# DeepBlender/DeepDenoiser

Hardware: AMD Instinct MI355X
Metric: train tiles/sec (128x128x32ch U-Net KPCN) (higher is better)
Workload: dtype bf16; 1 GPU; BASELINE config 2: U-Net [64,96,128]x4 + 5x5 KernelPrediction + 3-scale MultiScalePrediction, 32-channel render-pass stack, 128x128 tiles, full training step (fwd+SMAPE loss+bwd+Adam); global_batch=128, parallelism=dp1, hipgraph=True, inputs=resident in HBM

## Files before the change

deepdenoiser_amd/csrc/dd_compose_stream.h:

```cpp
#pragma once
#include "dd_common.h"
#include <type_traits>

namespace {

typedef __attribute__((ext_vector_type(16))) float f32x16_t;
typedef __attribute__((ext_vector_type(2))) unsigned int cs_u32x2;

template <typename T> __device__ __forceinline__ f32x16_t mma32(uint4 a, uint4 b, f32x16_t c);
template <> __device__ __forceinline__ f32x16_t mma32<bf16_t>(uint4 a, uint4 b, f32x16_t c) {
  return __builtin_amdgcn_mfma_f32_32x32x16_bf16(__builtin_bit_cast(bf16x8_t, a), __builtin_bit_cast(bf16x8_t, b), c, 0, 0, 0);
}
template <> __device__ __forceinline__ f32x16_t mma32<f16_t>(uint4 a, uint4 b, f32x16_t c) {
  return __builtin_amdgcn_mfma_f32_32x32x16_f16(__builtin_bit_cast(f16x8_t, a), __builtin_bit_cast(f16x8_t, b), c, 0, 0, 0);
}

typedef __attribute__((ext_vector_type(4))) unsigned int cs_u32x4;
template <typename T> __device__ __forceinline__ f32x16_t mma32_zero(uint4 a, uint4 b);
template <> __device__ __forceinline__ f32x16_t mma32_zero<bf16_t>(uint4 a, uint4 b) {
  f32x16_t d;
  const cs_u32x4 av = {a.x, a.y, a.z, a.w}, bv = {b.x, b.y, b.z, b.w};
  asm volatile("v_mfma_f32_32x32x16_bf16 %0, %1, %2, 0" : "=&v"(d) : "v"(av), "v"(bv));
  return d;
}
template <> __device__ __forceinline__ f32x16_t mma32_zero<f16_t>(uint4 a, uint4 b) {
  f32x16_t d;
  const cs_u32x4 av = {a.x, a.y, a.z, a.w}, bv = {b.x, b.y, b.z, b.w};
  asm volatile("v_mfma_f32_32x32x16_f16 %0, %1, %2, 0" : "=&v"(d) : "v"(av), "v"(bv));
  return d;
}

template <typename T> __device__ __forceinline__ void unpack2(uint32_t w, float& lo, float& hi);
template <> __device__ __forceinline__ void unpack2<bf16_t>(uint32_t w, float& lo, float& hi) { lo = __uint_as_float(w << 16); hi = __uint_as_float(w & 0xffff0000u); }
template <> __device__ __forceinline__ void unpack2<f16_t>(uint32_t w, float& lo, float& hi) { unpack_f16x2(w, lo, hi); }
template <typename T> __device__ __forceinline__ uint32_t packo(float lo, float hi) {
  uint32_t w = pack2<T>(lo, hi);
  asm("" : "+v"(w));
  return w;
}
template <typename T> struct One;
template <> struct One<bf16_t> { static constexpr uint32_t v = 0x3f80u; };
template <> struct One<f16_t> { static constexpr uint32_t v = 0x3c00u; };

__device__ __forceinline__ float dpp_xor1(float v) { return __int_as_float(__builtin_amdgcn_update_dpp(0, __float_as_int(v), 0xB1, 0xF, 0xF, true)); }
__device__ __forceinline__ void both_halves(float v, float& lower, float& upper) {
  const cs_u32x2 r = __builtin_amdgcn_permlane32_swap(__float_as_uint(v), __float_as_uint(v), false, false);
  lower = __uint_as_float(r[0]); upper = __uint_as_float(r[1]);
}

constexpr int PIXB = 48;

struct Unit { int b, yb0, yb1, xs, xe, fx0; };

template <typename P>
__device__ __forceinline__ void decode_unit(const P& p, int u, Unit& U) {
  const int j = u % p.nb, t = u / p.nb;
  const int st = t % p.n_strips;
  U.b = t / p.n_strips;
  U.yb0 = j * p.BH; U.yb1 = min(p.H, U.yb0 + p.BH);
  U.xs = st * p.SO; U.xe = min(p.W, U.xs + p.SO);
  U.fx0 = p.n_strips > 1 ? U.xs - 4 : 0;
}

struct Cursor {
  int urel, i;
  Unit U;
  template <typename P>
  __device__ __forceinline__ void init(const P& p, int u0, int nunits, int V) {
    urel = V >= 0 ? V / p.VB : -1 - ((-V - 1) / p.VB);
    i = V - urel * p.VB;
    U = Unit{0, 0, 0, 0, 0, 0};
    if (urel >= 0 && urel < nunits) decode_unit(p, u0 + urel, U);
  }
  template <typename P>
  __device__ __forceinline__ void advance(const P& p, int u0, int nunits, int rows) {
    i += rows;
    while (i >= p.VB) {
      i -= p.VB;
      ++urel;
      if (urel >= 0 && urel < nunits) decode_unit(p, u0 + urel, U);
    }
  }
};

__device__ __forceinline__ int sfl(int v) { return __builtin_amdgcn_readfirstlane(v); }
__device__ __forceinline__ int opaque(int v) { asm volatile("" : "+v"(v)); return v; }
__device__ __forceinline__ int posmod(int v, int d) { const int m = v % d; return m < 0 ? m + d : m; }

template <typename T> __device__ __forceinline__ float split3(float v, int e) {
  const float hi = Elem<T>::to_f32(Elem<T>::from_f32(v));
  const float mid = Elem<T>::to_f32(Elem<T>::from_f32(v - hi));
  const float lo = Elem<T>::to_f32(Elem<T>::from_f32(v - hi - mid));
  return e == 0 ? hi : e == 1 ? mid : lo;
}

}
```

deepdenoiser_amd/csrc/dd_compose_stream.hip:

```cpp
#include "dd_compose_stream.h"

#ifdef CS_PROFILE
__device__ unsigned long long cs_phase[4][8];
#define CSP_DECL() unsigned long long csp_last = __builtin_readcyclecounter(); const bool csp_on = blockIdx.x == 0 && t == 0 && lane == 0
#define CSP(i) do { const unsigned long long now_ = __builtin_readcyclecounter(); if (csp_on) cs_phase[LAYER][i] += now_ - csp_last; csp_last = now_; } while (0)
extern "C" int dd_debug_cs_phases(unsigned long long* out32, int reset) {
  if (out32) (void)hipMemcpyFromSymbol(out32, HIP_SYMBOL(cs_phase), sizeof(unsigned long long) * 32);
  if (reset) { unsigned long long z[32] = {0}; (void)hipMemcpyToSymbol(HIP_SYMBOL(cs_phase), z, sizeof(z)); }
  return 0;
}
#else
#define CSP_DECL()
#define CSP(i)
#endif


namespace {

constexpr int KS_MAX = 16;
constexpr int AUX_BYTES = 16 + 3 * 1024;

struct CsP {
  const float* small; const float* fine; float* out;
  const float* w_in; const float* b_in; const float* w_res[4]; const float* b_res[4]; const float* w_out; const float* b_out;
  void* save_act[5]; void* save_wl; void* save_netin;
  int ld_small, ld_fine, ld_out, ld_act[5], ld_wl, ld_netin;
  int N, H, W;
  int FW, R, TPR;
  int n_strips, SO;
  int BH, nb, VB;
  int units;
};

template <typename T>
__device__ __forceinline__ void stage_weights(char* img, char* aux, const CsP& p, int tid) {
  for (int i = tid; i < 4 * KS_MAX * 64 * 8; i += 1024) {
    const int e = i & 7, ln = (i >> 3) & 63, c = (i >> 9) & (KS_MAX - 1), l = i >> 13;
    const int m = ln & 31, g = 2 * c + (ln >> 5);
    float v = 0.f;
    if (m < 24) {
      if (g < 27) v = p.w_res[l][((g / 3) * 24 + 8 * (g % 3) + e) * 24 + m];
      else if (g == 27) { if (e < 3) v = split3<T>(p.b_res[l][m], e); }
    }
    reinterpret_cast<T*>(img)[i] = Elem<T>::from_f32(v);
  }
  T* ax = reinterpret_cast<T*>(aux);
  for (int i = tid; i < 8 + 3 * 512; i += 1024) {
    float v = 0.f;
    if (i < 8) v = i < 3 ? 1.f : 0.f;
    else {
      const int j = i - 8, e = j & 7, ln = (j >> 3) & 63, which = j >> 9;
      const int m = ln & 31, h = ln >> 5;
      if (which == 0) { if (m == 0) v = p.w_out[e < 4 ? 4 * h + e : 8 + 4 * h + e - 4]; }
      else if (which == 1) { if (m == 0) v = e < 4 ? p.w_out[16 + 4 * h + e] : (e < 7 && h == 0) ? split3<T>(p.b_out[0], e - 4) : 0.f; }
      else if (m < 24) v = e < 3 ? p.w_in[((h ? 0 : 3) + e) * 24 + m] : (e < 6 && h == 0) ? split3<T>(p.b_in[m], e - 3) : 0.f;
    }
    ax[i] = Elem<T>::from_f32(v);
  }
}

template <typename T, int LAYER, bool SAVE, int NPRE>
__device__ __forceinline__ void cs_role(const CsP& p, char* smem, char* aux, int ring_bytes, int t, int lane, int u0, int nunits, int steps) {
  constexpr bool RESIDUAL = LAYER == 1 || LAYER == 3;
  constexpr bool FINAL = LAYER == 3;
  constexpr int KS = 14;
  constexpr uint32_t ONE = One<T>::v, ONE2 = ONE | (ONE << 16);
  const int R = p.R, TPR = p.TPR, FW = p.FW, VB = p.VB;
  const int n = lane & 31, h = lane >> 5;
  const int r = t / TPR, xc = t - r * TPR;
  const bool has_task = t < R * TPR;
  const int x = xc * 32 + n;
  const int pitch = (FW + 2) * PIXB, rp = R * pitch;
  const int D0 = 3 * R + 2, D1 = 2 * R + 2, D4 = 3 * R + 2;
  const int off1 = D0 * pitch, off2 = off1 + D1 * pitch, off3 = off2 + D1 * pitch, off4 = off3 + D1 * pitch;
  const int Din = LAYER == 0 ? D0 : D1;
  const int Dres = LAYER == 1 ? D0 : D4;
  const int in_bytes = Din * pitch, out_bytes = D1 * pitch, res_bytes = Dres * pitch, raw_bytes = D4 * pitch;
  char* rin = smem + (LAYER == 0 ? 0 : LAYER == 1 ? off1 : LAYER == 2 ? off2 : off3);
  char* rout = smem + (LAYER == 0 ? off1 : LAYER == 1 ? off2 : off3);
  char* rres = smem + (LAYER == 1 ? 0 : off4);

  uint4 wa[KS];
#pragma unroll
  for (int c = 0; c < KS; ++c) wa[c] = *reinterpret_cast<const uint4*>(smem + ((LAYER * KS_MAX + c) * 64 + lane) * 16);
  __syncthreads();
  for (int i = threadIdx.x; i < ring_bytes / 16; i += 1024) reinterpret_cast<uint4*>(smem)[i] = uint4{0u, 0u, 0u, 0u};

  const int H = p.H, W = p.W, h2 = H >> 1, w2 = W >> 1;
  const int lag = (LAYER + 1) * (R + 1);
  const int total_rows = nunits * VB;
  const int s_beg = has_task ? (lag - r + R - 1) / R : steps, s_end = has_task ? (total_rows + lag - r + R - 1) / R : steps;
  Cursor cur;
  cur.init(p, u0, nunits, r - lag);
  int o_in = posmod(r - lag, Din) * pitch, o_out = posmod(r - lag, D1) * pitch, o_res = posmod(r - lag, Dres) * pitch, o_raw = posmod(r - lag, D4) * pitch;
  auto wrap_add = [](int o, int add, int bytes) { o += add; return o >= bytes ? o - bytes : o; };
  const int xo = x * PIXB + h * 16;
  const int a4c = h ? x * PIXB : x * PIXB + 128;
  const int a13c = h ? (int)(aux - rin) : x * PIXB + 128;
  const int wr = (x + 1) * PIXB + h * 8;
  int ybase = 0, pixb = 0;
  bool col_in = false, col_own = false, cols_all_in = false;
  auto unit_values = [&](const Cursor& c, int& yb, int& pb, bool& ci, bool& co, bool& call) {
    const int gx = c.U.fx0 + x;
    yb = c.U.yb0 - 4;
    ci = (unsigned)gx < (unsigned)W;
    co = ci && gx >= c.U.xs && gx < c.U.xe;
    pb = c.U.b * H * W + (ci ? gx : 0);
    call = c.U.fx0 + xc * 32 >= 0 && c.U.fx0 + xc * 32 + 32 <= W;
  };
  unit_values(cur, ybase, pixb, col_in, col_own, cols_all_in);

  Cursor c0;
  int o0 = 0, ybase0 = 0, pixb0 = 0, pix0 = 0;
  bool col_in0 = false, col_own0 = false, cols_all_in0 = false, in0 = false, own0 = false, row_in0 = false;
  float xin[3] = {0.f, 0.f, 0.f};
  const int s0_end = has_task ? (total_rows - r + R - 1) / R : 0;
  auto load_x0 = [&](int s_next) {
    in0 = false; own0 = false; row_in0 = false;
    if (s_next < s0_end) {
      const int y = ybase0 + c0.i;
      row_in0 = (unsigned)y < (unsigned)H;
      in0 = row_in0 && col_in0;
      own0 = in0 && col_own0 && y >= c0.U.yb0 && y < c0.U.yb1;
      const int cy = row_in0 ? y : 0;
      pix0 = pixb0 + cy * W;
      const int cx = pix0 - (c0.U.b * H + cy) * W;
      const float* src = h ? p.small + (size_t)((c0.U.b * h2 + (cy >> 1)) * w2 + (cx >> 1)) * p.ld_small : p.fine + (size_t)pix0 * p.ld_fine;
#ifdef CS_EXP_NO_STAGE0_LOADS
      xin[0] = (float)pix0; xin[1] = 1.f; xin[2] = 0.5f;
      (void)src;
#else
      xin[0] = src[0]; xin[1] = src[1]; xin[2] = src[2];
#endif
    }
  };
  if (LAYER == 0) {
    c0.init(p, u0, nunits, r);
    o0 = posmod(r, D0) * pitch;
    unit_values(c0, ybase0, pixb0, col_in0, col_own0, cols_all_in0);
    load_x0(0);
  }

  f32x16_t acc;
  auto conv_part_n = [&](auto pre_t) {
    constexpr bool pre = decltype(pre_t)::value;
    constexpr int C0 = pre ? 0 : NPRE, C1 = pre ? NPRE : KS;
    const int o_m1 = o_in == 0 ? in_bytes - pitch : o_in - pitch;
    const int o_p1 = o_in + pitch == in_bytes ? 0 : o_in + pitch;
    const char* q0 = rin + xo + o_m1;
    const char* q1 = rin + xo + 16 + o_in;
    const char* q2 = rin + xo + o_p1;
    const char* q4 = rin + a4c + (h ? o_in : o_m1);
    const char* q13 = rin + a13c + (h ? 0 : o_p1);
    f32x16_t c_init = {0.f, 0.f, 0.f, 0.f, 0.f, 0.f, 0.f, 0.f, 0.f, 0.f, 0.f, 0.f, 0.f, 0.f, 0.f, 0.f};
    if (RESIDUAL && pre) {
      const char* qr = rres + o_res + wr;
      uint2 rv[3];
#pragma unroll
      for (int b = 0; b < 3; ++b) rv[b] = *reinterpret_cast<const uint2*>(qr + b * 16);
#pragma unroll
      for (int b = 0; b < 3; ++b) {
        float r0, r1, r2, r3;
        unpack2<T>(rv[b].x, r0, r1); unpack2<T>(rv[b].y, r2, r3);
        c_init[4 * b] = r0; c_init[4 * b + 1] = r1; c_init[4 * b + 2] = r2; c_init[4 * b + 3] = r3;
      }
    }
    constexpr int BATCH = 6;
#pragma unroll
    for (int c0_ = C0; c0_ < C1; c0_ += BATCH) {
      uint4 bf[BATCH];
#pragma unroll
      for (int c = c0_; c < c0_ + BATCH && c < C1; ++c) {
        const char* a = c < 4 ? q0 + 32 * c : c == 4 ? q4 : c < 9 ? q1 + 32 * (c - 5) : c < 13 ? q2 + 32 * (c - 9) : q13;
#ifdef CS_EXP_NO_LDSREAD
        bf[c - c0_] = uint4{(uint32_t)x, (uint32_t)c, 0u, 0u};
#else
        bf[c - c0_] = *reinterpret_cast<const uint4*>(a);
#endif
      }
      __builtin_amdgcn_sched_barrier(0);
#pragma unroll
      for (int c = c0_; c < c0_ + BATCH && c < C1; ++c) {
#ifdef CS_EXP_NO_MFMA
        acc[c] = ((pre && c == 0) ? c_init[c] : acc[c]) + __uint_as_float(bf[c - c0_].x ^ wa[c].x);
#else
        acc = mma32<T>(wa[c], bf[c - c0_], (pre && c == 0) ? c_init : acc);
#endif
      }
      __builtin_amdgcn_sched_barrier(0);
    }
    if (pre && NPRE == 0) acc = c_init;
  };

  bool act = 0 >= s_beg && 0 < s_end;
  if (act) conv_part_n(std::true_type());

  CSP_DECL();
  for (int s = 0; s < steps; ++s) {
    CSP(0);
#ifndef CS_EXP_NO_BARRIER
    __syncthreads();
#endif
    CSP(1);
    if (LAYER == 0) {
      if (s < s0_end) {
        const uint4 w0 = *reinterpret_cast<const uint4*>(aux + 16 + 2048 + lane * 16);
        const uint4 bx = {pack2<T>(xin[0], xin[1]), pack2<T>(xin[2], h ? 0.f : 1.f), h ? 0u : ONE2, 0u};
        const f32x16_t z = {0.f, 0.f, 0.f, 0.f, 0.f, 0.f, 0.f, 0.f, 0.f, 0.f, 0.f, 0.f, 0.f, 0.f, 0.f, 0.f};
        const f32x16_t a0 = mma32<T>(w0, bx, z);
        char* o = rin + o0 + wr;
        const bool in_now = in0, own_now = own0, all_in = row_in0 && cols_all_in0;
        const int pix_now = pix0;
        if (SAVE && own_now && p.save_netin) {
          T* d = reinterpret_cast<T*>(p.save_netin) + (size_t)pix_now * p.ld_netin + (h ? 0 : 3);
#pragma unroll
          for (int e = 0; e < 3; ++e) d[e] = Elem<T>::from_f32(xin[e]);
          if (!h) { d[3] = Elem<T>::from_f32(0.f); d[4] = Elem<T>::from_f32(0.f); }
        }
        uint2 pk[3];
#pragma unroll
        for (int b = 0; b < 3; ++b) {
          pk[b].x = relu_bf16x2(packo<T>(a0[4 * b], a0[4 * b + 1]));
          pk[b].y = relu_bf16x2(packo<T>(a0[4 * b + 2], a0[4 * b + 3]));
        }
        if (!all_in) {
#pragma unroll
          for (int b = 0; b < 3; ++b) { pk[b].x = in_now ? pk[b].x : 0u; pk[b].y = in_now ? pk[b].y : 0u; }
        }
#pragma unroll
        for (int b = 0; b < 3; ++b) {
          *reinterpret_cast<uint2*>(o + b * 16) = pk[b];
          if (SAVE && own_now && p.save_act[0])
            *reinterpret_cast<uint2*>(reinterpret_cast<char*>(p.save_act[0]) + ((size_t)pix_now * p.ld_act[0] + 8 * b + 4 * h) * 2) = pk[b];
        }
      }
      c0.i += R;
      if (c0.i >= VB) {
        c0.i -= R;
        c0.advance(p, u0, nunits, R);
        unit_values(c0, ybase0, pixb0, col_in0, col_own0, cols_all_in0);
      }
      o0 = wrap_add(o0, rp, D0 * pitch);
      load_x0(s + 1);
    }
    CSP(2);
    if (act) {
      const int y = ybase + cur.i;
      const bool row_in = (unsigned)y < (unsigned)H;
      const bool all_in = row_in && cols_all_in;
      const bool inside = row_in && col_in;
      const bool own = inside && col_own && y >= cur.U.yb0 && y < cur.U.yb1;
      const int cy = row_in ? y : 0;
      const int pix = pixb + cy * W;
      float f3[3] = {0.f, 0.f, 0.f}, s3[3] = {0.f, 0.f, 0.f};
      if (FINAL) {
#ifndef CS_EXP_NO_TAIL_LOADS
        const int cx = pix - (cur.U.b * H + cy) * W;
        const float* fr = p.fine + (size_t)(pix + (h - (cy & 1)) * W) * p.ld_fine;
        const float* sp = p.small + (size_t)((cur.U.b * h2 + (cy >> 1)) * w2 + (cx >> 1)) * p.ld_small;
#pragma unroll
        for (int c = 0; c < 3; ++c) { f3[c] = fr[c]; s3[c] = sp[c]; }
#endif
      }
      conv_part_n(std::false_type());
      CSP(4);
      uint4 wo1 = {0u, 0u, 0u, 0u}, wo2 = {0u, 0u, 0u, 0u};
      if (FINAL) {
        wo1 = *reinterpret_cast<const uint4*>(aux + 16 + lane * 16);
        wo2 = *reinterpret_cast<const uint4*>(aux + 16 + 1024 + lane * 16);
      }
      uint2 pk[3];
#pragma unroll
      for (int b = 0; b < 3; ++b) {
        pk[b].x = packo<T>(acc[4 * b], acc[4 * b + 1]);
        pk[b].y = packo<T>(acc[4 * b + 2], acc[4 * b + 3]);
      }
      if (!FINAL) {
        if (LAYER == 1) {
          char* o4 = smem + off4 + o_raw + wr;
          if (!all_in) {
#pragma unroll
            for (int b = 0; b < 3; ++b) { pk[b].x = inside ? pk[b].x : 0u; pk[b].y = inside ? pk[b].y : 0u; }
          }
#pragma unroll
          for (int b = 0; b < 3; ++b) {
            *reinterpret_cast<uint2*>(o4 + b * 16) = pk[b];
            if (SAVE && own && p.save_act[2])
              *reinterpret_cast<uint2*>(reinterpret_cast<char*>(p.save_act[2]) + ((size_t)pix * p.ld_act[2] + 8 * b + 4 * h) * 2) = pk[b];
          }
        }
#pragma unroll
        for (int b = 0; b < 3; ++b) { pk[b].x = relu_bf16x2(pk[b].x); pk[b].y = relu_bf16x2(pk[b].y); }
        if (LAYER != 1 && !all_in) {
#pragma unroll
          for (int b = 0; b < 3; ++b) { pk[b].x = inside ? pk[b].x : 0u; pk[b].y = inside ? pk[b].y : 0u; }
        }
        char* o = rout + o_out + wr;
#pragma unroll
        for (int b = 0; b < 3; ++b) {
          *reinterpret_cast<uint2*>(o + b * 16) = pk[b];
          if (SAVE && LAYER != 1 && own && p.save_act[LAYER + 1])
            *reinterpret_cast<uint2*>(reinterpret_cast<char*>(p.save_act[LAYER + 1]) + ((size_t)pix * p.ld_act[LAYER + 1] + 8 * b + 4 * h) * 2) = pk[b];
        }
      } else {
#ifdef CS_EXP_NO_TAIL
        if (own && h == 0 && pk[0].x == 0x12345u) p.out[(size_t)pix * p.ld_out] = 1.f;
#else
        if (SAVE && own && p.save_act[4]) {
#pragma unroll
          for (int b = 0; b < 3; ++b)
            *reinterpret_cast<uint2*>(reinterpret_cast<char*>(p.save_act[4]) + ((size_t)pix * p.ld_act[4] + 8 * b + 4 * h) * 2) = pk[b];
        }
        const f32x16_t z = {0.f, 0.f, 0.f, 0.f, 0.f, 0.f, 0.f, 0.f, 0.f, 0.f, 0.f, 0.f, 0.f, 0.f, 0.f, 0.f};
        f32x16_t a2 = mma32<T>(wo1, uint4{pk[0].x, pk[0].y, pk[1].x, pk[1].y}, z);
        a2 = mma32<T>(wo2, uint4{pk[2].x, pk[2].y, ONE2, ONE}, a2);
        const uint32_t wlp = pack2<T>(fmaxf(a2[0], 0.f), 0.f);
        float wlv, unused;
        unpack2<T>(wlp, wlv, unused);
        const float wgt = 1.f / (1.f + __expf(-wlv));
        float res[3];
#pragma unroll
        for (int c = 0; c < 3; ++c) {
          const float pair = f3[c] + dpp_xor1(f3[c]);
          float p_lo, p_hi, f_lo, f_hi;
          both_halves(pair, p_lo, p_hi);
          both_halves(f3[c], f_lo, f_hi);
          const float low = 0.25f * (p_lo + p_hi);
          const float fme = (cy & 1) ? f_hi : f_lo;
          res[c] = fme - wgt * low + wgt * s3[c];
        }
        if (own && h == 0) {
          float* o = p.out + (size_t)pix * p.ld_out;
#pragma unroll
          for (int c = 0; c < 3; ++c) o[c] = res[c];
          if (SAVE && p.save_wl) reinterpret_cast<uint16_t*>(p.save_wl)[(size_t)pix * p.ld_wl] = (uint16_t)(wlp & 0xffffu);
        }
#endif
      }
    }
    CSP(5);
    cur.i += R;
    if (cur.i >= VB) {
      cur.i -= R;
      cur.advance(p, u0, nunits, R);
      unit_values(cur, ybase, pixb, col_in, col_own, cols_all_in);
    }
    o_in = wrap_add(o_in, rp, in_bytes);
    if (!FINAL) o_out = wrap_add(o_out, rp, out_bytes);
    if (RESIDUAL) o_res = wrap_add(o_res, rp, res_bytes);
    if (LAYER == 1) o_raw = wrap_add(o_raw, rp, raw_bytes);
    act = s + 1 >= s_beg && s + 1 < s_end;
    if (act) conv_part_n(std::true_type());
    CSP(6);
  }
}

template <typename T, bool SAVE, bool R1>
__global__ __launch_bounds__(1024) void compose_stream_fwd_kernel(const CsP p) {
  extern __shared__ __attribute__((aligned(16))) char smem[];
  const int tid = threadIdx.x, lane = tid & 63, wave = sfl(tid >> 6);
  const int rows = 12 * p.R + 10;
  const int ring_bytes = rows * (p.FW + 2) * PIXB;
  char* aux = smem + ring_bytes;
  stage_weights<T>(smem, aux, p, tid);
  const int G = gridDim.x, g = blockIdx.x;
  const int u0 = (int)(((long)p.units * g) / G), u1 = (int)(((long)p.units * (g + 1)) / G);
  const int nunits = u1 - u0;
  const int steps = nunits > 0 ? (nunits * p.VB + 4 * (p.R + 1) + p.R - 1) / p.R : 0;
  const int layer = wave >> 2, t = wave & 3;
  __syncthreads();
  const int r = t / p.TPR;
#define CS_ROLE(L)                                                                                   \
  do {                                                                                               \
    if (R1 || r == 0) cs_role<T, L, SAVE, 9>(p, smem, aux, ring_bytes, t, lane, u0, nunits, steps);  \
    else if (r == 1) cs_role<T, L, SAVE, 4>(p, smem, aux, ring_bytes, t, lane, u0, nunits, steps);   \
    else cs_role<T, L, SAVE, 0>(p, smem, aux, ring_bytes, t, lane, u0, nunits, steps);               \
  } while (0)
  if (layer == 0) CS_ROLE(0);
  else if (layer == 1) CS_ROLE(1);
  else if (layer == 2) CS_ROLE(2);
  else CS_ROLE(3);
#undef CS_ROLE
}

}

extern "C" int dd_compose_stream_plan(int N, int H, int W, int cus, int* out8) {
  if (N <= 0 || H <= 0 || W <= 0 || cus <= 0 || !out8) return DD_ERR_INVALID;
  int n_strips = 1, SO = W, FW = ((W + 31) / 32) * 32;
  if (W > 128) {
    for (n_strips = 2;; ++n_strips) {
      SO = (W + n_strips - 1) / n_strips;
      SO += SO & 1;
      FW = ((SO + 8 + 31) / 32) * 32;
      if (FW <= 128) break;
    }
  }
  const int R = FW == 32 ? 4 : FW == 64 ? 2 : 1;
  long best = -1; int bestBH = 0;
  for (int d = 1; d <= 16; ++d) {
    int BH = (H + d - 1) / d;
    BH = ((BH + 3) / 4) * 4;
    if (BH < 4) BH = 4;
    const int nb = (H + BH - 1) / BH;
    const long units = (long)N * n_strips * nb;
    const long G = units < cus ? units : cus;
    const long per = (units + G - 1) / G;
    const long cost = per * (BH + 8) + 4 * (R + 1);
    if (best < 0 || cost < best) { best = cost; bestBH = BH; }
  }
  const int nb = (H + bestBH - 1) / bestBH;
  out8[0] = FW; out8[1] = R; out8[2] = FW / 32; out8[3] = n_strips; out8[4] = SO; out8[5] = bestBH; out8[6] = nb; out8[7] = bestBH + 8;
  return DD_OK;
}

int dd_compose_stream_fwd_launch(const dd_compose_args* a, hipStream_t s) {
  CsP p;
  p.small = a->small; p.fine = a->fine; p.out = a->out;
  p.w_in = a->w_in; p.b_in = a->b_in; p.w_out = a->w_out; p.b_out = a->b_out;
  for (int l = 0; l < 4; ++l) { p.w_res[l] = a->w_res[l]; p.b_res[l] = a->b_res[l]; }
  bool save = a->save_wl != nullptr;
  for (int i = 0; i < 5; ++i) { p.save_act[i] = a->save_act[i]; p.ld_act[i] = a->ld_act[i]; save = save || a->save_act[i]; }
  p.save_wl = a->save_wl; p.ld_wl = a->ld_wl;
  p.save_netin = a->save_netin; p.ld_netin = a->ld_netin; save = save || a->save_netin;
  p.ld_small = a->ld_small; p.ld_fine = a->ld_fine; p.ld_out = a->ld_out;
  p.N = a->N; p.H = a->H; p.W = a->W;
  DD_REQUIRE((long)a->N * a->H * a->W < (1l << 31) / 64, "dd_compose_net_fwd: N * H * W = %ld pixels exceed the 32-bit offsets of the kernel", (long)a->N * a->H * a->W);
  const int cus = dd_device_cus();
  int g8[8];
  if (dd_compose_stream_plan(a->N, a->H, a->W, cus, g8) != DD_OK) return DD_ERR_INVALID;
  p.FW = g8[0]; p.R = g8[1]; p.TPR = g8[2]; p.n_strips = g8[3]; p.SO = g8[4]; p.BH = g8[5]; p.nb = g8[6]; p.VB = g8[7];
  p.units = a->N * p.n_strips * p.nb;
  const int grid = p.units < cus ? p.units : cus;
  const int lds = (12 * p.R + 10) * (p.FW + 2) * PIXB + AUX_BYTES;
#define CS_LAUNCH(T, SV, R1)                                                                          \
  do {                                                                                                \
    dd_allow_max_lds(reinterpret_cast<const void*>(compose_stream_fwd_kernel<T, SV, R1>));            \
    hipLaunchKernelGGL((compose_stream_fwd_kernel<T, SV, R1>), dim3(grid), dim3(1024), lds, s, p);    \
  } while (0)
#define CS_LAUNCH_R(T, SV) do { if (p.R == 1) CS_LAUNCH(T, SV, true); else CS_LAUNCH(T, SV, false); } while (0)
  if (a->dtype == DD_BF16) { if (save) CS_LAUNCH_R(bf16_t, true); else CS_LAUNCH_R(bf16_t, false); }
  else { if (save) CS_LAUNCH_R(f16_t, true); else CS_LAUNCH_R(f16_t, false); }
#undef CS_LAUNCH_R
#undef CS_LAUNCH
  DD_LAUNCH_CHECK();
  return DD_OK;
}
```

Baseline: 16110 tiles/s.

## Widen activation saves via permlane swap and prefetch tail loads earlier

Activation saves now go through a helper that uses permlane32_swap so each half-wave writes one 16-byte store instead of two 8-byte stores per pixel for the first two channel blocks. The final layer's fine and small image loads are issued before the pre-part of the next step's convolution, so their global-memory latency overlaps with MFMA work. The final layer's pre-part batch size drops to 3, and the act[4] save moves after the tail computation. Compile-time experiment macros to disable saves are also added. Register pressure rises because the f3/s3 values are now live across the loop.

```diff
diff --git a/deepdenoiser_amd/csrc/dd_compose_stream.h b/deepdenoiser_amd/csrc/dd_compose_stream.h
--- a/deepdenoiser_amd/csrc/dd_compose_stream.h
+++ b/deepdenoiser_amd/csrc/dd_compose_stream.h
@@ -50,6 +50,20 @@
 
 constexpr int PIXB = 48;
 
+__device__ __forceinline__ void store_pixel24(bool pred, char* px, int h, uint2 pk0, uint2 pk1, uint2 pk2) {
+  const cs_u32x2 sx = __builtin_amdgcn_permlane32_swap(pk0.x, pk1.x, false, false);
+  const cs_u32x2 sy = __builtin_amdgcn_permlane32_swap(pk0.y, pk1.y, false, false);
+  if (pred) {
+#ifdef CS_EXP_NARROW_SAVES
+    *reinterpret_cast<uint2*>(px + 8 * h) = pk0;
+    *reinterpret_cast<uint2*>(px + 16 + 8 * h) = pk1;
+#else
+    *reinterpret_cast<uint4*>(px + 16 * h) = uint4{sx[0], sy[0], sx[1], sy[1]};
+#endif
+    *reinterpret_cast<uint2*>(px + 32 + 8 * h) = pk2;
+  }
+}
+
 struct Unit { int b, yb0, yb1, xs, xe, fx0; };
 
 template <typename P>
diff --git a/deepdenoiser_amd/csrc/dd_compose_stream.hip b/deepdenoiser_amd/csrc/dd_compose_stream.hip
--- a/deepdenoiser_amd/csrc/dd_compose_stream.hip
+++ b/deepdenoiser_amd/csrc/dd_compose_stream.hip
@@ -12,6 +12,12 @@
 #else
 #define CSP_DECL()
 #define CSP(i)
+#endif
+
+#ifdef CS_EXP_NO_SAVES
+#define CS_SAVING(word) ((word) == 0x7fc12345u)
+#else
+#define CS_SAVING(word) true
 #endif
 
 
@@ -165,7 +171,7 @@
         c_init[4 * b] = r0; c_init[4 * b + 1] = r1; c_init[4 * b + 2] = r2; c_init[4 * b + 3] = r3;
       }
     }
-    constexpr int BATCH = 6;
+    constexpr int BATCH = (pre && FINAL) ? 3 : 6;
 #pragma unroll
     for (int c0_ = C0; c0_ < C1; c0_ += BATCH) {
       uint4 bf[BATCH];
@@ -192,8 +198,25 @@
     if (pre && NPRE == 0) acc = c_init;
   };
 
+  float f3[3] = {0.f, 0.f, 0.f}, s3[3] = {0.f, 0.f, 0.f};
+  auto request_tail = [&]() {
+#ifndef CS_EXP_NO_TAIL_LOADS
+    const int y = ybase + cur.i;
+    const int cy = (unsigned)y < (unsigned)H ? y : 0;
+    const int pix = pixb + cy * W;
+    const int cx = pix - (cur.U.b * H + cy) * W;
+    const float* fr = p.fine + (size_t)(pix + (h - (cy & 1)) * W) * p.ld_fine;
+    const float* sp = p.small + (size_t)((cur.U.b * h2 + (cy >> 1)) * w2 + (cx >> 1)) * p.ld_small;
+#pragma unroll
+    for (int c = 0; c < 3; ++c) { f3[c] = fr[c]; s3[c] = sp[c]; }
+#endif
+  };
+
   bool act = 0 >= s_beg && 0 < s_end;
-  if (act) conv_part_n(std::true_type());
+  if (act) {
+    if (FINAL) request_tail();
+    conv_part_n(std::true_type());
+  }
 
   CSP_DECL();
   for (int s = 0; s < steps; ++s) {
@@ -211,7 +234,7 @@
         char* o = rin + o0 + wr;
         const bool in_now = in0, own_now = own0, all_in = row_in0 && cols_all_in0;
         const int pix_now = pix0;
-        if (SAVE && own_now && p.save_netin) {
+        if (SAVE && own_now && p.save_netin && CS_SAVING(__float_as_uint(xin[0]))) {
           T* d = reinterpret_cast<T*>(p.save_netin) + (size_t)pix_now * p.ld_netin + (h ? 0 : 3);
 #pragma unroll
           for (int e = 0; e < 3; ++e) d[e] = Elem<T>::from_f32(xin[e]);
@@ -230,9 +253,8 @@
 #pragma unroll
         for (int b = 0; b < 3; ++b) {
           *reinterpret_cast<uint2*>(o + b * 16) = pk[b];
-          if (SAVE && own_now && p.save_act[0])
-            *reinterpret_cast<uint2*>(reinterpret_cast<char*>(p.save_act[0]) + ((size_t)pix_now * p.ld_act[0] + 8 * b + 4 * h) * 2) = pk[b];
-        }
+        }
+        if (SAVE) store_pixel24(own_now && p.save_act[0] && CS_SAVING(pk[0].x), reinterpret_cast<char*>(p.save_act[0]) + (size_t)pix_now * p.ld_act[0] * 2, h, pk[0], pk[1], pk[2]);
       }
       c0.i += R;
       if (c0.i >= VB) {
@@ -252,16 +274,6 @@
       const bool own = inside && col_own && y >= cur.U.yb0 && y < cur.U.yb1;
       const int cy = row_in ? y : 0;
       const int pix = pixb + cy * W;
-      float f3[3] = {0.f, 0.f, 0.f}, s3[3] = {0.f, 0.f, 0.f};
-      if (FINAL) {
-#ifndef CS_EXP_NO_TAIL_LOADS
-        const int cx = pix - (cur.U.b * H + cy) * W;
-        const float* fr = p.fine + (size_t)(pix + (h - (cy & 1)) * W) * p.ld_fine;
-        const float* sp = p.small + (size_t)((cur.U.b * h2 + (cy >> 1)) * w2 + (cx >> 1)) * p.ld_small;
-#pragma unroll
-        for (int c = 0; c < 3; ++c) { f3[c] = fr[c]; s3[c] = sp[c]; }
-#endif
-      }
       conv_part_n(std::false_type());
       CSP(4);
       uint4 wo1 = {0u, 0u, 0u, 0u}, wo2 = {0u, 0u, 0u, 0u};
@@ -285,9 +297,8 @@
 #pragma unroll
           for (int b = 0; b < 3; ++b) {
             *reinterpret_cast<uint2*>(o4 + b * 16) = pk[b];
-            if (SAVE && own && p.save_act[2])
-              *reinterpret_cast<uint2*>(reinterpret_cast<char*>(p.save_act[2]) + ((size_t)pix * p.ld_act[2] + 8 * b + 4 * h) * 2) = pk[b];
           }
+          if (SAVE) store_pixel24(own && p.save_act[2] && CS_SAVING(pk[0].x), reinterpret_cast<char*>(p.save_act[2]) + (size_t)pix * p.ld_act[2] * 2, h, pk[0], pk[1], pk[2]);
         }
 #pragma unroll
         for (int b = 0; b < 3; ++b) { pk[b].x = relu_bf16x2(pk[b].x); pk[b].y = relu_bf16x2(pk[b].y); }
@@ -299,18 +310,13 @@
 #pragma unroll
         for (int b = 0; b < 3; ++b) {
           *reinterpret_cast<uint2*>(o + b * 16) = pk[b];
-          if (SAVE && LAYER != 1 && own && p.save_act[LAYER + 1])
-            *reinterpret_cast<uint2*>(reinterpret_cast<char*>(p.save_act[LAYER + 1]) + ((size_t)pix * p.ld_act[LAYER + 1] + 8 * b + 4 * h) * 2) = pk[b];
-        }
+        }
+        if (SAVE && LAYER != 1)
+          store_pixel24(own && p.save_act[LAYER + 1] && CS_SAVING(pk[0].x), reinterpret_cast<char*>(p.save_act[LAYER + 1]) + (size_t)pix * p.ld_act[LAYER + 1] * 2, h, pk[0], pk[1], pk[2]);
       } else {
 #ifdef CS_EXP_NO_TAIL
         if (own && h == 0 && pk[0].x == 0x12345u) p.out[(size_t)pix * p.ld_out] = 1.f;
 #else
-        if (SAVE && own && p.save_act[4]) {
-#pragma unroll
-          for (int b = 0; b < 3; ++b)
-            *reinterpret_cast<uint2*>(reinterpret_cast<char*>(p.save_act[4]) + ((size_t)pix * p.ld_act[4] + 8 * b + 4 * h) * 2) = pk[b];
-        }
         const f32x16_t z = {0.f, 0.f, 0.f, 0.f, 0.f, 0.f, 0.f, 0.f, 0.f, 0.f, 0.f, 0.f, 0.f, 0.f, 0.f, 0.f};
         f32x16_t a2 = mma32<T>(wo1, uint4{pk[0].x, pk[0].y, pk[1].x, pk[1].y}, z);
         a2 = mma32<T>(wo2, uint4{pk[2].x, pk[2].y, ONE2, ONE}, a2);
@@ -333,7 +339,12 @@
           float* o = p.out + (size_t)pix * p.ld_out;
 #pragma unroll
           for (int c = 0; c < 3; ++c) o[c] = res[c];
-          if (SAVE && p.save_wl) reinterpret_cast<uint16_t*>(p.save_wl)[(size_t)pix * p.ld_wl] = (uint16_t)(wlp & 0xffffu);
+          if (SAVE && p.save_wl && CS_SAVING(wlp)) reinterpret_cast<uint16_t*>(p.save_wl)[(size_t)pix * p.ld_wl] = (uint16_t)(wlp & 0xffffu);
+        }
+        if (SAVE && own && p.save_act[4] && CS_SAVING(pk[0].x)) {
+#pragma unroll
+          for (int b = 0; b < 3; ++b)
+            *reinterpret_cast<uint2*>(reinterpret_cast<char*>(p.save_act[4]) + ((size_t)pix * p.ld_act[4] + 8 * b + 4 * h) * 2) = pk[b];
         }
 #endif
       }
@@ -350,7 +361,10 @@
     if (RESIDUAL) o_res = wrap_add(o_res, rp, res_bytes);
     if (LAYER == 1) o_raw = wrap_add(o_raw, rp, raw_bytes);
     act = s + 1 >= s_beg && s + 1 < s_end;
-    if (act) conv_part_n(std::true_type());
+    if (act) {
+      if (FINAL) request_tail();
+      conv_part_n(std::true_type());
+    }
     CSP(6);
   }
 }
```

New measurement: 16120 tiles/s, median of 3. Within noise of the previous version (+0.1%).
